# buttomnutstoast/Multigrid-Neural-Architectures

Hardware: NVIDIA B200
Metric: R-MG-34 train images/sec (higher is better)
Workload: dtype bf16

## Files before the change

include/mgconv.h:

```cpp
#ifndef MGCONV_H
#define MGCONV_H

#include <stdint.h>
#include <stddef.h>

#ifdef __cplusplus
extern "C" {
#endif

enum {
  MG_MAX_SEG = 6,
  MG_MAX_SRC = 8
};

typedef struct mg_ctx mg_ctx;

typedef enum {
  MG_OK = 0,
  MG_ERR_INVALID_ARG = 1,
  MG_ERR_SHAPE = 2,
  MG_ERR_CUDA = 3,
  MG_ERR_NCCL = 4,
  MG_ERR_UNSUPPORTED = 5
} mg_status;

typedef enum { MG_F32 = 0, MG_BF16 = 1 } mg_dtype;

typedef enum {
  MG_SEG_SAME = 0,
  MG_SEG_POOL = 1,
  MG_SEG_UP = 2
} mg_seg_mode;

typedef enum { MG_IMPL_AUTO = 0, MG_IMPL_SIMT = 1, MG_IMPL_TCGEN05 = 2 } mg_impl;

typedef struct { int64_t hi, lo; } mg_sum;

typedef struct {
  void* data;
  const float* scale;
  const float* shift;
  int32_t relu;
  int32_t N, H, W, C, Cp;
} mg_grid;

typedef struct {
  int32_t n_seg;
  mg_grid seg[MG_MAX_SEG];
  int32_t seg_mode[MG_MAX_SEG];
  int32_t ksize, stride, pad;
  int32_t Cout;
  int32_t H, W;
  int32_t algo_fwd, algo_bwd_data;
} mg_conv_desc;
enum { MG_ALGO_AUTO = 0, MG_ALGO_TILE128 = 1,
       MG_ALGO_TILE256 = 2,
       MG_ALGO_RESIDENT = 3,
       MG_ALGO_TILE128_DEEP = 4,
       MG_ALGO_TILE256_DEEP = 5,
       MG_ALGO_TILE128_MID = 6,
       MG_ALGO_PAIR128 = 7,
       MG_ALGO_PAIR256 = 8,
       MG_ALGO_RESIDENT_PAIR = 9 };

typedef struct {
  mg_grid g;
  int32_t c_offset;
  int32_t mode;
  const void* aux;
} mg_grad_src;

int mg_ctx_create(int device, void* cuda_stream, int dtype, mg_ctx** out);
int mg_ctx_destroy(mg_ctx* ctx);
int mg_ctx_set_stream(mg_ctx* ctx, void* cuda_stream);
int mg_ctx_set_impl(mg_ctx* ctx, int impl);
int mg_ctx_lane(mg_ctx* ctx, int lane);
int mg_ctx_event_record(mg_ctx* ctx, int ev);
int mg_ctx_event_wait(mg_ctx* ctx, int ev);
int mg_ctx_sync(mg_ctx* ctx);
enum { MG_TUNE_HALO_SUBTILES = 0,
       MG_TUNE_PERSISTENT = 1,
       MG_TUNE_STEM_FUSED_STATS = 2  };
int mg_ctx_set_tuning(mg_ctx* ctx, int knob, int value);
const char* mg_last_error(mg_ctx* ctx);
int mg_version(void);
int mg_ctx_launch_count(mg_ctx* ctx, int64_t* out);
int mg_ctx_tc_launch_count(mg_ctx* ctx, int64_t* out);
int mg_ctx_profile(mg_ctx* ctx, int on);
int mg_ctx_profile_read(mg_ctx* ctx, double* conv_ms, int64_t* conv_calls);

int mg_import_nchw(mg_ctx* ctx, const float* src, mg_grid* dst);
int mg_export_nchw(mg_ctx* ctx, const mg_grid* src, float* dst);

int mg_crop_flip_normalize(mg_ctx* ctx, const float* src, int32_t N, int32_t C, int32_t H, int32_t W, float* dst, int32_t oH, int32_t oW,
                           const int32_t* y0, const int32_t* x0, const int32_t* flip, const float* mean, const float* stdv);

size_t mg_conv_packed_bytes(const mg_conv_desc* d, int transposed);
int mg_conv_pack_weights(mg_ctx* ctx, const mg_conv_desc* d, const float* w, void* wpack, int transposed);
int mg_conv_pack_weights_batched(mg_ctx* ctx, int32_t n, const mg_conv_desc* const* descs, const float* const* w,
                                 void* const* wpack, const int32_t* transposed);

int mg_conv_forward(mg_ctx* ctx, const mg_conv_desc* d, const float* w, const void* wpack,
                    const float* bias, mg_grid* y, mg_sum* bn_sums);

int mg_bn_finalize(mg_ctx* ctx, const mg_sum* bn_sums, int64_t count, int32_t C, int32_t Cp,
                   const float* gamma, const float* beta, float* running_mean, float* running_var,
                   float eps, float momentum, int training,
                   float* scale, float* shift, float* save_mean, float* save_invstd);

int mg_residual_forward(mg_ctx* ctx, const mg_grid* z, const mg_grid* s, int relu, mg_grid* out, mg_grid* pooled);

typedef struct {
  const mg_sum* sums;
  int64_t count;
  const float* gamma;
  const float* beta;
// ... 89 lines not shown
```

multigrid-neural-architectures_b200/csrc/umma_conv.cu:

```cuda
#include "common.cuh"
#include "conv_view.cuh"
#include "umma_common.cuh"
#include "tma.cuh"
#include <algorithm>
#include <vector>

namespace {

constexpr int BM = 128;
constexpr int KV_PER_STAGE = 8;
constexpr int A_STAGE_BYTES = BM * 128;
constexpr int N_PRODUCERS = 128;
constexpr int MMA_WARP = 4, B_WARP = 5;
constexpr int N_THREADS = 192;
constexpr int MAX_STAGES = 8;

struct UParams {
  USeg seg[MG_MAX_SEG];
  int n_seg;
  int k, stride, pad;
  int H, W;
  int Ho, Wo;
  int64_t M;
  int Nimg;
// ... 266 lines not shown
      if (leader) tc_commit(&tmem_full_bar);
    }
  }
  __syncthreads();
  if (warp == MMA_WARP) {
    tc_fence_after();
    asm volatile("tcgen05.dealloc.cta_group::1.sync.aligned.b32 %0, %1;" ::"r"(tmem_base), "r"(p.tmem_cols) : "memory");
  }
}



__device__ __forceinline__ float warp_reduce_scatter16(float (&v)[16], int lane) {
#pragma unroll
  for (int o = 8; o >= 1; o >>= 1) {
    const bool hi = (lane & o) != 0;
#pragma unroll
    for (int i = 0; i < o; ++i) {
      const float send = hi ? v[i] : v[i + o];
      const float keep = hi ? v[i + o] : v[i];
      v[i] = keep + __shfl_xor_sync(0xffffffffu, send, o);
    }
  }
  return v[0] + __shfl_xor_sync(0xffffffffu, v[0], 16);
}

constexpr int MAX_CHUNKS = 32;
struct HChunk { int seg, c0, nch, tps, ksteps, stage0; };

struct HParams {
  CUtensorMap tmap[MG_MAX_SEG];
  int seg_up[MG_MAX_SEG];
  HChunk chunk[MAX_CHUNKS];
  int n_seg, n_chunks, n_stages, any_up;
  int img_box;
  int H, W, Wp, Hp, Nimg;
  int64_t T;
  int HL;
  int nr_max;
  int halo_bytes;
  int n_abuf;
  int n_tile;
  const uint8_t* wpack;
  const float* bias;
  int c_bias;
  __nv_bfloat16* y;
  int y_pitch, c_valid;
  int stages, tmem_cols;
  mg_sum* stats;
  int c_stats;
  int m_tiles;
  CUtensorMap tmap_w;
  int tile_rows;
  int epi_stage;
};

__device__ __forceinline__ void zero_pad_column(uint8_t* a_smem, int nbuf, int halo_bytes, int nr_max, int Wp, int tid, int nthreads, int org = 0) {
  for (int i = tid; i < nbuf * nr_max * 8; i += nthreads) {
    const int q = i & 7, row = (i >> 3) % nr_max, buf = (i >> 3) / nr_max;
    *reinterpret_cast<uint4*>(a_smem + (size_t)buf * halo_bytes + (size_t)(org + row * Wp + Wp - 1) * 128 + q * 16) = make_uint4(0, 0, 0, 0);
  }
  fence_proxy_async();
}

__device__ __forceinline__ void zero_halo_margins(uint8_t* a_smem, int nbuf, int halo_bytes, int HL, int Wp, int tid, int nthreads) {
  const int m = Wp + 1;
  for (int i = tid; i < nbuf * 2 * m * 8; i += nthreads) {
    const int q = i & 7, sl = (i >> 3) % (2 * m), buf = (i >> 3) / (2 * m);
    const int slot = sl < m ? sl : HL - 2 * m + sl;
    *reinterpret_cast<uint4*>(a_smem + (size_t)buf * halo_bytes + (size_t)slot * 128 + q * 16) = make_uint4(0, 0, 0, 0);
  }
  fence_proxy_async();
}

__device__ __forceinline__ bool slot_pixel(const HParams& p, int64_t t, uint32_t* pix) {
  if (t >= p.T) return false;
  const uint32_t tu = (uint32_t)t, spi = (uint32_t)(p.Hp * p.Wp);
  const uint32_t n = tu / spi, rem = tu - n * spi;
  const uint32_t yy = rem / (uint32_t)p.Wp, xs = rem - yy * (uint32_t)p.Wp;
  if ((int)yy >= p.H || (int)xs >= p.W) return false;
  *pix = (n * p.H + yy) * p.W + xs;
  return true;
}

template <int MT>
__global__ void __launch_bounds__(32 * (4 * MT + 3), MT == 1 ? 4 : 2) umma_conv_halo_kernel(const __grid_constant__ HParams p) {
  constexpr int EPI_WARPS = 4 * MT, A_WARP = EPI_WARPS, B_WARP = EPI_WARPS + 1, M_WARP = EPI_WARPS + 2, NT = 32 * (EPI_WARPS + 3);
  extern __shared__ __align__(1024) uint8_t smem_raw[];
  uint8_t* smem = (uint8_t*)(((uintptr_t)smem_raw + 1023) & ~(uintptr_t)1023);
  __shared__ uint64_t full_bar[MAX_STAGES], empty_bar[MAX_STAGES], a_full[2], a_empty[2], tmem_full_bar;
  __shared__ uint32_t tmem_base_s;
  __shared__ float s_bias[256];

  pdl_launch();
  const int tid = threadIdx.x, warp = tid >> 5, lane = tid & 31;
  const int S = p.stages;
  const int b_stage_bytes = p.n_tile * 128;
  uint8_t* a_smem = smem;
  uint8_t* b_smem = smem + (size_t)p.n_abuf * p.halo_bytes;
  const int t0 = (int)blockIdx.x * (BM * MT);
  const int ntile = blockIdx.y;
  const int hs = t0 - p.Wp - 1;
  const int r0 = floordiv(hs, p.Wp);
  const int nr = (hs + p.HL - 1) / p.Wp - r0 + 1;
  const int off = p.img_box ? 0 : hs - r0 * p.Wp;

// ... 319 lines not shown
      }
    }
  } else if (rank == 0) {
    const bool leader = elect_one();
    const uint32_t idesc = (1u << 4) | (1u << 7) | (1u << 10) | ((uint32_t)(p.n_tile >> 3) << 17) | ((uint32_t)(256 >> 4) << 24);
    Ring ra(p.n_abuf), rb(S);
    for (int c = 0; c < p.n_chunks; ++c, ra.next()) {
      const int buf = ra.idx;
      const HChunk ch = p.chunk[c];
      mbar_wait_cluster(&a_full[buf], ra.phase);
      tc_fence_after();
      const uint32_t a_base = smem_u32(a_smem + (size_t)buf * p.halo_bytes) + (uint32_t)a_first * 128u;
      const int tps = ch.tps, ksteps = ch.ksteps;
      const uint32_t sub_lo = 8u / (uint32_t)tps;
      int sub = 0;
      uint32_t b_lo = 0;
      for (int tap = 0; tap < 9; ++tap) {
        if (sub == 0) {
          mbar_wait_cluster(&full_bar[rb.idx], rb.phase);
          tc_fence_after();
          b_lo = desc_lo_k_sw128(smem_u32(b_smem + (size_t)rb.idx * b_half_bytes));
        }
        const uint32_t a_lo = desc_lo_k_sw128(a_base + (uint32_t)((tap / 3) * p.Wp + (tap % 3)) * 128u);
        const bool last_of_stage = (sub == tps - 1) || tap == 8;
        if (leader) {
#pragma unroll
          for (int mt = 0; mt < MT; ++mt)
#pragma unroll
            for (int q = 0; q < 4; ++q)
              if (q < ksteps) {
                tc_mma_bf16_lohi_pair(tmem_base + (uint32_t)(mt * p.n_tile), a_lo + (uint32_t)(mt * BM * 8 + q * 2), b_lo + (uint32_t)sub * sub_lo + (uint32_t)(q * 2),
                                      DESC_HI_SW128, idesc, (uint32_t)((c | tap | q) != 0));
              }
          if (last_of_stage) tc_commit_pair(&empty_bar[rb.idx]);
        }
        if (last_of_stage) { sub = 0; rb.next(); } else ++sub;
      }
      if (leader) tc_commit_pair(&a_empty[buf]);
    }
    if (leader) tc_commit_pair(&tmem_full_bar);
  }
  __syncthreads();
  cluster_sync_all();
  if (warp == M_WARP) {
    tc_fence_after();
    asm volatile("tcgen05.dealloc.cta_group::2.sync.aligned.b32 %0, %1;" ::"r"(tmem_base), "r"(p.tmem_cols) : "memory");
  }
}


constexpr int P_A_WARP = 8, P_B_WARP = 9, P_MMA_WARP = 10, P_THREADS = 352;
constexpr int P_MAX_ABUF = 6;

__global__ void __launch_bounds__(P_THREADS, 1) umma_conv_halo_persistent_kernel(const __grid_constant__ HParams p) {
  pdl_launch();
  extern __shared__ __align__(1024) uint8_t smem_raw[];
  uint8_t* smem = (uint8_t*)(((uintptr_t)smem_raw + 1023) & ~(uintptr_t)1023);
  __shared__ uint64_t b_full, a_full[P_MAX_ABUF], a_empty[P_MAX_ABUF], tmem_full[2], tmem_empty[2];
  __shared__ uint32_t tmem_base_s;

  const int tid = threadIdx.x, warp = tid >> 5, lane = tid & 31;
  const int NA = p.n_abuf;
  const int b_stage_bytes = p.n_tile * 128;
  uint8_t* a_smem = smem;
  uint8_t* b_smem = smem + (size_t)NA * p.halo_bytes;
  long long* s_part = reinterpret_cast<long long*>(b_smem + (size_t)p.n_stages * b_stage_bytes);
  float* s_bias = reinterpret_cast<float*>(s_part + 32 * p.n_tile);
  const int n_my = (p.m_tiles - (int)blockIdx.x + (int)gridDim.x - 1) / (int)gridDim.x;
  const int R = p.tile_rows;
  const int tile_slots = R ? R * p.Wp : BM;

  for (int c = tid; c < 32 * p.n_tile; c += P_THREADS) s_part[c] = 0;
  if (tid == 0) {
    mbar_init(&b_full, 1);
    for (int s = 0; s < NA; ++s) { mbar_init(&a_full[s], 1); mbar_init(&a_empty[s], 1); }
    for (int s = 0; s < 2; ++s) { mbar_init(&tmem_full[s], 1); mbar_init(&tmem_empty[s], 128); }
    asm volatile("fence.mbarrier_init.release.cluster;" ::: "memory");
  }
  if (warp == P_MMA_WARP) {
    asm volatile("tcgen05.alloc.cta_group::1.sync.aligned.shared::cta.b32 [%0], %1;" ::"r"(smem_u32(&tmem_base_s)), "r"(p.tmem_cols)
                 : "memory");
    asm volatile("tcgen05.relinquish_alloc_permit.cta_group::1.sync.aligned;" ::: "memory");
  }
  if (warp == P_A_WARP && lane < p.n_seg) tma_prefetch_desc(&p.tmap[lane]);
  if (p.img_box) zero_halo_margins(a_smem, NA, p.halo_bytes, p.HL, p.Wp, tid, P_THREADS);
  else if (p.any_up) zero_pad_column(a_smem, NA, p.halo_bytes, p.nr_max, p.Wp, tid, P_THREADS, R ? 1 : 0);
  if (R) {
    for (int i = tid; i < NA * 2 * 8; i += P_THREADS) {
      const int q = i & 7, which = (i >> 3) & 1, buf = i >> 4;
      const int slot = which ? 1 + (R + 2) * p.Wp : 0;
      *reinterpret_cast<uint4*>(a_smem + (size_t)buf * p.halo_bytes + (size_t)slot * 128 + q * 16) = make_uint4(0, 0, 0, 0);
    }
    fence_proxy_async();
  }
  pdl_wait();
  for (int c = tid; c < p.n_tile; c += P_THREADS) s_bias[c] = (p.bias && c < p.c_bias) ? p.bias[c] : 0.f;
  tc_fence_before();
  __syncthreads();
  tc_fence_after();
  const uint32_t tmem_base = tmem_base_s;

  if (warp < 8) {
    const int grp = warp >> 2, qw = warp & 3;
    const bool want_stats = p.stats != nullptr;
#ifdef MG_PHASE_PROF
    long long e_wait = 0, e_work = 0;
#endif
    for (int it = grp; it < n_my; it += 2) {
      const int mt = blockIdx.x + it * gridDim.x;
      const int acc = it & 1;
      const int row = qw * 32 + lane;
      uint32_t pix = 0;
      const bool row_ok = row < tile_slots && slot_pixel(p, (int64_t)mt * tile_slots + row, &pix);
#ifdef MG_PHASE_PROF
      const long long e0 = clock64();
#endif
      mbar_wait(&tmem_full[acc], (it >> 1) & 1);
      tc_fence_after();
#ifdef MG_PHASE_PROF
      const long long e1 = clock64();
#endif
      __nv_bfloat16* yrow = p.y + (size_t)pix * p.y_pitch;
      const uint32_t tcol = tmem_base + ((uint32_t)(qw * 32) << 16) + (uint32_t)(acc * p.n_tile);
      for (int c0 = 0; c0 < p.n_tile; c0 += 16) {
        uint32_t a16[16];
        tc_ld16(tcol + (uint32_t)c0, a16);
        tc_wait_ld();
        uint32_t pk[2][4];
#pragma unroll
        for (int h = 0; h < 2; ++h) {
          const int n0 = c0 + h * 8;
#pragma unroll
          for (int e = 0; e < 4; ++e) {
            const float a = __uint_as_float(a16[h * 8 + 2 * e]) + s_bias[c0 + h * 8 + 2 * e];
            const float b = __uint_as_float(a16[h * 8 + 2 * e + 1]) + s_bias[c0 + h * 8 + 2 * e + 1];
            __nv_bfloat162 t2 = __floats2bfloat162_rn(a, b);
            pk[h][e] = *reinterpret_cast<uint32_t*>(&t2);
          }
          if (row_ok && n0 + 8 <= p.c_valid) *reinterpret_cast<uint4*>(yrow + n0) = make_uint4(pk[h][0], pk[h][1], pk[h][2], pk[h][3]);
        }
        if (want_stats) {
#pragma unroll
          for (int h = 0; h < 2; ++h) {
            const bool use = row_ok && c0 + h * 8 + 8 <= p.c_valid;
            float sv[16];
#pragma unroll
            for (int e = 0; e < 4; ++e) {
              const float ra = use ? __uint_as_float(pk[h][e] << 16) : 0.f, rb = use ? __uint_as_float(pk[h][e] & 0xFFFF0000u) : 0.f;
              sv[2 * e] = ra; sv[2 * e + 1] = rb;
              sv[8 + 2 * e] = ra * ra; sv[8 + 2 * e + 1] = rb * rb;
            }
            const float tot = warp_reduce_scatter16(sv, lane);
            if (lane < 16) {
              long long fh, fl;
              mg_to_fix_f32(tot, fh, fl);
              long long* sp = s_part + (size_t)((warp * 2 + (lane >> 3)) * p.n_tile + c0 + h * 8 + (lane & 7)) * 2;
              sp[0] += fh; sp[1] += fl;
            }
          }
        }
      }
      tc_fence_before();
      mbar_arrive(&tmem_empty[acc]);
#ifdef MG_PHASE_PROF
      e_wait += e1 - e0; e_work += clock64() - e1;
#endif
    }
#ifdef MG_PHASE_PROF
    if (blockIdx.x == 3 && tid == 0) printf("epilogue warp0: tiles %d wait_tmem_full %lld work %lld cycles/tile\n", n_my, e_wait / n_my, e_work / n_my);
#endif
    if (want_stats) {
      asm volatile("bar.sync 3, 256;" ::: "memory");
      for (int c = tid; c < p.n_tile; c += 256)
        if (c < p.c_stats) {
          long long ah = 0, al = 0, bh = 0, bl = 0;
#pragma unroll
          for (int w = 0; w < 8; ++w) {
            const long long* sa = s_part + (size_t)((w * 2) * p.n_tile + c) * 2;
            const long long* sb = s_part + (size_t)((w * 2 + 1) * p.n_tile + c) * 2;
            ah += sa[0]; al += sa[1]; bh += sb[0]; bl += sb[1];
          }
          mg_sum_add_fix(p.stats + c, ah, al);
          mg_sum_add_fix(p.stats + p.c_stats + c, bh, bl);
        }
    }
  } else if (warp == P_A_WARP) {
    Ring ra(NA);
    int ac = 0;
    for (int it = 0; it < n_my; ++it) {
      const int t0 = (int)(blockIdx.x + it * gridDim.x) * tile_slots;
      const int hs = t0 - p.Wp - 1;
      const int r0 = R ? t0 / p.Wp - 1 : floordiv(hs, p.Wp);
      const int nr = R ? R + 2 : (hs + p.HL - 1) / p.Wp - r0 + 1;
      for (int c = 0; c < p.n_chunks; ++c, ++ac, ra.next()) {
        const int buf = ra.idx;
        if (ac >= NA) mbar_wait(&a_empty[buf], ra.phase ^ 1u);
        const HChunk ch = p.chunk[c];
        const uint32_t dst = smem_u32(a_smem + (size_t)buf * p.halo_bytes) + (R ? 128u : 0u);
        if (p.img_box) tma_load_images(&p.tmap[ch.seg], dst + (uint32_t)(p.Wp + 1) * 128u, &a_full[buf], ch.c0, t0 / (p.Hp * p.Wp), (uint32_t)BM * 128u, lane);
        else tma_load_rows(&p.tmap[ch.seg], p.seg_up[ch.seg], dst, &a_full[buf], ch.c0, r0, nr, p.W, p.Hp, lane);
      }
    }
  } else if (warp == P_B_WARP) {
    if (lane == 0) {
      mbar_arrive_expect_tx(&b_full, (uint32_t)(p.n_stages * b_stage_bytes));
      for (int q = 0; q < p.n_stages; ++q)
        bulk_g2s(smem_u32(b_smem + (size_t)q * b_stage_bytes), p.wpack + (size_t)q * b_stage_bytes, (uint32_t)b_stage_bytes, &b_full);
    }
  } else {
    const bool leader = elect_one();
    const uint32_t idesc = idesc_bf16_m128(p.n_tile);
    const uint32_t b_base = smem_u32(b_smem);
    Ring ra(NA);
    mbar_wait(&b_full, 0);
#ifdef MG_PHASE_PROF
    long long m_wait_e = 0, m_wait_a = 0, m_issue = 0, m_t0 = clock64();
#endif
    for (int it = 0; it < n_my; ++it) {
      const int acc = it & 1;
#ifdef MG_PHASE_PROF
      const long long q0 = clock64();
#endif
      if (it >= 2) { mbar_wait(&tmem_empty[acc], ((it >> 1) - 1) & 1); tc_fence_after(); }
#ifdef MG_PHASE_PROF
      m_wait_e += clock64() - q0;
#endif
      const uint32_t d_tmem = tmem_base + (uint32_t)(acc * p.n_tile);
      const int t0 = (int)(blockIdx.x + it * gridDim.x) * tile_slots;
      const int hs = t0 - p.Wp - 1;
      const int off = (p.img_box || R) ? 0 : hs - floordiv(hs, p.Wp) * p.Wp;
      for (int c = 0; c < p.n_chunks; ++c, ra.next()) {
        const int buf = ra.idx;
        const HChunk ch = p.chunk[c];
#ifdef MG_PHASE_PROF
        const long long q1 = clock64();
#endif
        mbar_wait(&a_full[buf], ra.phase);
        tc_fence_after();
#ifdef MG_PHASE_PROF
        const long long q2 = clock64();
        m_wait_a += q2 - q1;
#endif
        const uint32_t a_base = smem_u32(a_smem + (size_t)buf * p.halo_bytes) + (uint32_t)off * 128u;
        const int tps = ch.tps, ksteps = ch.ksteps;
        const uint32_t sub_lo = 8u / (uint32_t)tps;
        if (leader) {
          int sub = 0, st = ch.stage0;
          for (int tap = 0; tap < 9; ++tap) {
            const uint32_t a_lo = desc_lo_k_sw128(a_base + (uint32_t)((tap / 3) * p.Wp + (tap % 3)) * 128u);
            const uint32_t b_lo = desc_lo_k_sw128(b_base + (uint32_t)(st * b_stage_bytes)) + (uint32_t)sub * sub_lo;
#pragma unroll
            for (int q = 0; q < 4; ++q)
              if (q < ksteps) tc_mma_bf16_lohi(d_tmem, a_lo + (uint32_t)(q * 2), b_lo + (uint32_t)(q * 2), DESC_HI_SW128, idesc, (uint32_t)((c | tap | q) != 0));
            if (++sub == tps) { sub = 0; ++st; }
          }
          tc_commit(&a_empty[buf]);
        }
#ifdef MG_PHASE_PROF
        m_issue += clock64() - q2;
#endif
      }
      if (leader) tc_commit(&tmem_full[acc]);
    }
#ifdef MG_PHASE_PROF
    if (blockIdx.x == 3 && lane == 0) printf("MMA warp: tiles %d total %lld wait_tmem_empty %lld wait_a_full %lld issue %lld cycles/tile\n", n_my, (clock64() - m_t0) / n_my, m_wait_e / n_my, m_wait_a / n_my, m_issue / n_my);
#endif
  }
  __syncthreads();
  if (warp == P_MMA_WARP) {
    tc_fence_after();
    asm volatile("tcgen05.dealloc.cta_group::1.sync.aligned.b32 %0, %1;" ::"r"(tmem_base), "r"(p.tmem_cols) : "memory");
  }
}


__global__ void __cluster_dims__(2, 1, 1) __launch_bounds__(P_THREADS, 1) umma_conv_halo_persistent_pair_kernel(const __grid_constant__ HParams p) {
  pdl_launch();
  extern __shared__ __align__(1024) uint8_t smem_raw[];
  uint8_t* smem = (uint8_t*)(((uintptr_t)smem_raw + 1023) & ~(uintptr_t)1023);
  __shared__ uint64_t b_full, a_full[P_MAX_ABUF], a_empty[P_MAX_ABUF], tmem_full[2], tmem_empty[2];
  __shared__ uint32_t tmem_base_s;
// ... 696 lines not shown
    p.stages = S;
    const int smem = p.n_abuf * p.halo_bytes + S * half + 1024;
    MG_REQUIRE(ctx, smem <= SMEM_MAX, MG_ERR_UNSUPPORTED, "pair halo conv: %d bytes of shared memory", smem);
    p.epi_stage = epilogue_staging(p, MT, smem - 1024);
    int rc = mg_tensor_map(ctx, p.wpack, g.n_tiles * p.n_stages * p.n_tile, 0, 0, 0, 5, p.n_tile / 2, &p.tmap_w);
    if (rc) return rc;
    static bool pair_attr_set = false;
    if (!pair_attr_set) {
      MG_CUDA(ctx, cudaFuncSetAttribute(umma_conv_halo_pair_kernel<1>, cudaFuncAttributeMaxDynamicSharedMemorySize, SMEM_MAX));
      MG_CUDA(ctx, cudaFuncSetAttribute(umma_conv_halo_pair_kernel<2>, cudaFuncAttributeMaxDynamicSharedMemorySize, SMEM_MAX));
      pair_attr_set = true;
    }
    dim3 grid((unsigned)mg_round_up((int)mg_cdiv(p.T, BM * MT), 2), (unsigned)g.n_tiles);
    if (MT == 2) MG_CUDA(ctx, mg_launch_pdl(umma_conv_halo_pair_kernel<2>, grid, dim3(32 * 11), (size_t)smem, ctx->stream, p));
    else MG_CUDA(ctx, mg_launch_pdl(umma_conv_halo_pair_kernel<1>, grid, dim3(32 * 7), (size_t)smem, ctx->stream, p));
    MG_CHECK_LAUNCH(ctx);
    ctx->tc_launches++;
    return MG_OK;
  }
  int budget_kb;
  if (MT == 1) {
    budget_kb = p.n_tile >= 192 ? 108 : 56;
  } else {
    const int ctas = std::max(1, std::min(512 / cols, 2));
    budget_kb = ctas == 1 ? 200 : 108;
  }
  if (algo == MG_ALGO_TILE128_MID) budget_kb = 72;
  if ((algo == MG_ALGO_AUTO || algo == MG_ALGO_RESIDENT) && mg_cdiv(p.T, BM * MT) * g.n_tiles <= ctx->num_sms) budget_kb = 200;
  if (algo == MG_ALGO_TILE128_DEEP) budget_kb = 108;
  if (algo == MG_ALGO_TILE256_DEEP) budget_kb = 200;
  if (budget_env > 0) budget_kb = budget_env;
  const int min_ring = 2;
  p.n_abuf = (g.n_chunks > 1 && 2 * p.halo_bytes + min_ring * b_stage <= budget_kb * 1024) ? 2 : 1;
  int S = (budget_kb * 1024 - p.n_abuf * p.halo_bytes) / b_stage;
  S = std::max(2, std::min(S, std::min(MAX_STAGES, p.n_stages)));
  p.stages = S;
  static bool attr_set = false;
  if (!attr_set) {
    MG_CUDA(ctx, cudaFuncSetAttribute(umma_conv_halo_kernel<1>, cudaFuncAttributeMaxDynamicSharedMemorySize, SMEM_MAX));
    MG_CUDA(ctx, cudaFuncSetAttribute(umma_conv_halo_kernel<2>, cudaFuncAttributeMaxDynamicSharedMemorySize, SMEM_MAX));
    attr_set = true;
  }
  const int smem = p.n_abuf * p.halo_bytes + S * b_stage + 1024;
  MG_REQUIRE(ctx, smem <= SMEM_MAX, MG_ERR_UNSUPPORTED, "halo conv: %d bytes of shared memory", smem);
  p.epi_stage = epilogue_staging(p, MT, smem - 1024);
  dim3 grid((unsigned)mg_cdiv(p.T, BM * MT), (unsigned)g.n_tiles);
  if (MT == 2) MG_CUDA(ctx, mg_launch_pdl(umma_conv_halo_kernel<2>, grid, dim3(32 * 11), (size_t)smem, ctx->stream, p));
  else MG_CUDA(ctx, mg_launch_pdl(umma_conv_halo_kernel<1>, grid, dim3(32 * 7), (size_t)smem, ctx->stream, p));
  MG_CHECK_LAUNCH(ctx);
  ctx->tc_launches++;
  return MG_OK;
}

struct PersistPlan { int n_abuf, smem, tmem_cols, grid, tile_rows, halo_bytes, pair; };
static int persist_tile_rows(const mg_conv_desc* d, int Nimg, bool any_up) {
  const int Wp = d->W + 1, Hp = d->H + 1;
  if (Wp > BM) return 0;
  if (!any_up && BM % (Hp * Wp) == 0) return 0;
  const int R = BM / Wp;
  if (R < 1 || R * Wp * 100 < BM * 85) return 0;
  (void)Nimg;
  return R;
}
static bool persist_plan(const mg_ctx* ctx, const mg_conv_desc* d, const Geometry& g, int Nimg, int algo, bool stats, PersistPlan* pl) {
  static int on = -1, min_tiles_per_sm = -1;
  if (on < 0) { const char* e = getenv("MGCONV_PERSIST"); on = e ? atoi(e) : 1; }
  if (min_tiles_per_sm < 0) { const char* e = getenv("MGCONV_PERSIST_MIN_TILES"); min_tiles_per_sm = e ? atoi(e) : 4; }
  if (algo == MG_ALGO_TILE128 || algo == MG_ALGO_TILE256 || algo == MG_ALGO_TILE128_DEEP || algo == MG_ALGO_TILE256_DEEP ||
      algo == MG_ALGO_TILE128_MID || algo == MG_ALGO_PAIR128 || algo == MG_ALGO_PAIR256) return false;
  const bool pair = algo == MG_ALGO_RESIDENT_PAIR;
  const bool forced = algo == MG_ALGO_RESIDENT || pair || ctx->tune_persist == 1;
  if (!forced && (ctx->tune_persist == 2 || !on)) return false;
  if (!g.halo || g.n_tiles != 1) return false;
  HParams hp;
  hp.Wp = d->W + 1; hp.img_box = 0;
  halo_geometry(hp, BM);
  bool any_up = false;
  for (int s = 0; s < d->n_seg; ++s) any_up = any_up || d->seg_mode[s] == MG_SEG_UP;
  static int aligned_single = -1;
  if (aligned_single < 0) { const char* e = getenv("MGCONV_PERSIST_ALIGNED"); aligned_single = e ? atoi(e) : 0; }
  const int R = ((pair || aligned_single) && !stats) ? persist_tile_rows(d, Nimg, any_up && g.n_chunks > 0) : 0;
  if (R) hp.halo_bytes = mg_round_up(((R + 2) * hp.Wp + 2) * 128, 1024);
  const int64_t m_tiles = R ? mg_cdiv((int64_t)Nimg * (d->H + 1), R) : mg_cdiv((int64_t)Nimg * (d->H + 1) * hp.Wp, BM);
  if (!forced && m_tiles < (int64_t)min_tiles_per_sm * ctx->num_sms) return false;
  if (pair && !R && !(!any_up && BM % ((d->H + 1) * hp.Wp) == 0)) return false;
  const int b_bytes = g.n_stages * g.n_tile * (pair ? 64 : 128);
  const int tail = g.n_tile * (4 + 256);
  const int room = SMEM_MAX - 1024 - b_bytes - tail;
  int n_abuf = room / hp.halo_bytes;
  if (n_abuf < 2) return false;
  n_abuf = std::min(n_abuf, std::min(P_MAX_ABUF, 2 * g.n_chunks + 1));
  int cols = 32;
  while (cols < 2 * g.n_tile) cols <<= 1;
  if (cols > 512) return false;
  pl->n_abuf = n_abuf; pl->smem = n_abuf * hp.halo_bytes + b_bytes + tail + 1024; pl->tmem_cols = cols;
  pl->grid = (int)std::min<int64_t>(m_tiles, ctx->num_sms);
  if (pair) pl->grid = 2 * (int)std::min<int64_t>((m_tiles + 1) / 2, ctx->num_sms / 2);
  pl->tile_rows = R; pl->halo_bytes = hp.halo_bytes; pl->pair = pair ? 1 : 0;
  return true;
}

static int launch_halo_persistent(mg_ctx* ctx, HParams& p, const PersistPlan& pl, const mg_grid* segs) {
  { int rc = halo_tensor_maps(ctx, p, segs, BM); if (rc) return rc; }
  halo_geometry(p, BM);
  p.m_tiles = (int)mg_cdiv(p.T, BM);
  p.tile_rows = p.img_box ? 0 : pl.tile_rows;
  if (p.tile_rows) {
    p.halo_bytes = pl.halo_bytes;
    p.nr_max = p.tile_rows + 2;
    p.m_tiles = (int)mg_cdiv((int64_t)p.Nimg * p.Hp, p.tile_rows);
  }
  p.tmem_cols = pl.tmem_cols;
  p.n_abuf = pl.n_abuf;
  p.stages = 0;
  static bool attr_set = false;
  if (!attr_set) {
    MG_CUDA(ctx, cudaFuncSetAttribute(umma_conv_halo_persistent_kernel, cudaFuncAttributeMaxDynamicSharedMemorySize, SMEM_MAX));
    attr_set = true;
  }
  if (pl.pair) {
    int rc = mg_tensor_map(ctx, p.wpack, p.n_stages * p.n_tile, 0, 0, 0, 5, p.n_tile / 2, &p.tmap_w);
    if (rc) return rc;
    static bool pair_attr = false;
    if (!pair_attr) {
      MG_CUDA(ctx, cudaFuncSetAttribute(umma_conv_halo_persistent_pair_kernel, cudaFuncAttributeMaxDynamicSharedMemorySize, SMEM_MAX));
      pair_attr = true;
    }
    MG_CUDA(ctx, mg_launch_pdl(umma_conv_halo_persistent_pair_kernel, dim3(pl.grid), dim3(P_THREADS), (size_t)pl.smem, ctx->stream, p));
    MG_CHECK_LAUNCH(ctx);
    ctx->tc_launches++;
    return MG_OK;
  }
  MG_CUDA(ctx, mg_launch_pdl(umma_conv_halo_persistent_kernel, dim3(pl.grid), dim3(P_THREADS), (size_t)pl.smem, ctx->stream, p));
  MG_CHECK_LAUNCH(ctx);
  ctx->tc_launches++;
  return MG_OK;
}

static bool fused_stats_on() {
  static int on = -1;
  if (on < 0) { const char* e = getenv("MGCONV_FUSED_STATS"); on = e ? atoi(e) : 1; }
  return on != 0;
}

static int fill_halo_params(mg_ctx* ctx, HParams& p, const Geometry& g, int n_seg, const mg_grid* segs, const int* up, int N, int H, int W) {
  memset(&p, 0, sizeof(p));
  p.n_seg = n_seg; p.n_chunks = g.n_chunks; p.n_stages = g.n_stages;
  for (int c = 0; c < g.n_chunks; ++c) p.chunk[c] = g.chunk[c];
  p.H = H; p.W = W; p.Wp = W + 1; p.Hp = H + 1; p.Nimg = N;
  p.T = (int64_t)N * p.Hp * p.Wp;
  p.n_tile = g.n_tile;
  for (int s = 0; s < n_seg; ++s) {
    p.seg_up[s] = up[s];
    if (up[s]) p.any_up = 1;
  }
  return MG_OK;
}

}

bool umma_wgrad_supported(const mg_ctx* ctx, const mg_conv_desc* d);

bool umma_conv_supported(const mg_ctx* ctx, const mg_conv_desc* d, int kind) {
  if (ctx->dtype != MG_BF16) return false;
  if (kind == 2) return umma_wgrad_supported(ctx, d);
  if (kind == 1 && d->stride != 1) return false;
// ... 195 lines not shown
```

multigrid-neural-architectures_b200/mgconv/ffi.py:

```python
import ctypes as C
import os

MG_MAX_SEG = 6
MG_MAX_SRC = 8
MG_F32, MG_BF16 = 0, 1
MG_SEG_SAME, MG_SEG_POOL, MG_SEG_UP, MG_SRC_POOL3 = 0, 1, 2, 3
MG_IMPL_AUTO, MG_IMPL_SIMT, MG_IMPL_TCGEN05 = 0, 1, 2
MG_TUNE_HALO_SUBTILES, MG_TUNE_PERSISTENT, MG_TUNE_STEM_FUSED_STATS = 0, 1, 2
MG_ALGO_AUTO, MG_ALGO_TILE128, MG_ALGO_TILE256, MG_ALGO_RESIDENT, MG_ALGO_TILE128_DEEP, MG_ALGO_TILE256_DEEP, MG_ALGO_TILE128_MID = 0, 1, 2, 3, 4, 5, 6
MG_ALGO_PAIR128, MG_ALGO_PAIR256, MG_ALGO_RESIDENT_PAIR = 7, 8, 9

_HERE = os.path.dirname(os.path.abspath(__file__))
LIB_PATH = os.environ.get("MGCONV_LIB", os.path.join(_HERE, "libmgconv.so"))


class MGError(RuntimeError):
    pass


class mg_grid(C.Structure):
    _fields_ = [("data", C.c_void_p), ("scale", C.c_void_p), ("shift", C.c_void_p), ("relu", C.c_int32),
                ("N", C.c_int32), ("H", C.c_int32), ("W", C.c_int32), ("C", C.c_int32), ("Cp", C.c_int32)]


class mg_conv_desc(C.Structure):
    _fields_ = [("n_seg", C.c_int32), ("seg", mg_grid * MG_MAX_SEG), ("seg_mode", C.c_int32 * MG_MAX_SEG),
                ("ksize", C.c_int32), ("stride", C.c_int32), ("pad", C.c_int32), ("Cout", C.c_int32),
                ("H", C.c_int32), ("W", C.c_int32), ("algo_fwd", C.c_int32), ("algo_bwd_data", C.c_int32)]


class mg_grad_src(C.Structure):
    _fields_ = [("g", mg_grid), ("c_offset", C.c_int32), ("mode", C.c_int32), ("aux", C.c_void_p)]


MG_STAGE_MAX_GRIDS = 4


class mg_stage_desc(C.Structure):
    _fields_ = [("n_scales", C.c_int32), ("C_in", C.c_int32 * MG_STAGE_MAX_GRIDS), ("C_out", C.c_int32 * MG_STAGE_MAX_GRIDS),
                ("H", C.c_int32 * MG_STAGE_MAX_GRIDS), ("W", C.c_int32 * MG_STAGE_MAX_GRIDS), ("ksize", C.c_int32 * MG_STAGE_MAX_GRIDS),
                ("residual", C.c_int32), ("no_final_relu", C.c_int32), ("eps", C.c_float), ("momentum", C.c_float)]


class mg_stage_params(C.Structure):
    _fields_ = [(name, C.c_void_p * (2 * MG_STAGE_MAX_GRIDS)) for name in
                ("conv_w", "conv_b", "bn_g", "bn_b", "bn_rm", "bn_rv", "conv_gw", "conv_gb", "bn_gg", "bn_gb")]


class mg_bn_fused(C.Structure):
    _fields_ = [("sums", C.c_void_p), ("count", C.c_int64), ("gamma", C.c_void_p), ("beta", C.c_void_p),
                ("running_mean", C.c_void_p), ("running_var", C.c_void_p), ("eps", C.c_float), ("momentum", C.c_float),
                ("training", C.c_int32), ("save_mean", C.c_void_p), ("save_invstd", C.c_void_p)]


def _load():
    if not os.path.exists(LIB_PATH):
        raise MGError(
            f"{LIB_PATH} not found: build it with `make -C multigrid-neural-architectures_b200/csrc` "
            "(or __graft_entry__.build()); there is no CPU / PyTorch fallback for the multigrid hot path")
    return C.CDLL(LIB_PATH, mode=C.RTLD_GLOBAL)


lib = _load()
# ... 135 lines not shown
```

multigrid-neural-architectures_b200/mgconv/ops.py:

```python
import ctypes as C
import os
import torch

from . import ffi
from .ffi import mg_grid, mg_conv_desc, mg_grad_src, mg_bn_fused, ptr, MG_SEG_SAME, MG_SEG_POOL, MG_SEG_UP, MG_SRC_POOL3, MG_MAX_SRC


def cpad(c):
    return (c + 7) // 8 * 8


def _k(x):
    if x is None:
        return None
    if isinstance(x, torch.Tensor):
        return x.data_ptr()
    if isinstance(x, mg_grid):
        return x.data
    return int(x)


def _keys(*xs):
    return [k for k in (_k(x) for x in xs) if k]

# ... 176 lines not shown
        d = mg_conv_desc()
        d.n_seg = len(self.segs)
        for i, (t, m) in enumerate(self.segs):
            d.seg[i] = t.grid()
            d.seg_mode[i] = m
        d.ksize, d.stride, d.pad, d.Cout, d.H, d.W = self.k, self.stride, self.pad, self.Cout, self.H, self.W
        self.desc = d
        self.y.buf = E.alloc(self.y.shape())
        self.yg = self.y.grid()
        if self.want_stats:
            self.sums = E.alloc_sums(2 * self.Cout, "fwd")
        t0 = self.segs[0][0]
        self.col = None
        if (E.use_packed and len(self.segs) == 1 and self.segs[0][1] == MG_SEG_SAME and self.stride > 1 and self.k > 1
                and t0.C * self.k * self.k <= 512 and not t0.needs_grad and os.environ.get("MGCONV_STEM_IM2COL", "0") == "1"):
            K = t0.C * self.k * self.k
            Kp = cpad(K)
            self.col = E.alloc((self.y.N, self.Ho, self.Wo, Kp))
            self.col_g = mg_grid(self.col.data_ptr(), None, None, 0, self.y.N, self.Ho, self.Wo, K, Kp)
            self.in_g = t0.grid()
            d1 = mg_conv_desc()
            d1.n_seg = 1
            d1.seg[0] = self.col_g
            d1.seg_mode[0] = MG_SEG_SAME
            d1.ksize, d1.stride, d1.pad, d1.Cout, d1.H, d1.W = 1, 1, 0, self.Cout, self.Ho, self.Wo
            self.desc_direct, self.desc = d, d1
        self.wpack = self.wpack_t = None
        nb = ffi.lib.mg_conv_packed_bytes(C.byref(self.desc), 0) if E.use_packed else 0
        if nb:
            self.wpack = E.alloc((nb,), torch.uint8)
        self.Ccat = sum(t.C for t, _ in self.segs)
        self.CcatP = sum(t.Cp for t, _ in self.segs)

    def pack(self, E):
        if self.wpack is not None:
            E.ctx.call("mg_conv_pack_weights", C.byref(self.desc), ptr(self.mod.weight), ptr(self.wpack), 0)
        if self.wpack_t is not None:
            E.ctx.call("mg_conv_pack_weights", C.byref(self.desc), ptr(self.mod.weight), ptr(self.wpack_t), 1)

    def pack_jobs(self):
        jobs = []
        if self.wpack is not None:
            jobs.append((self.desc, self.mod.weight, self.wpack, 0))
        if self.wpack_t is not None:
            jobs.append((self.desc, self.mod.weight, self.wpack_t, 1))
        return jobs

    def _tunable(self):
        return self.wpack is not None and self.k == 3 and self.stride == 1 and self.pad == 1 and 7 <= self.W <= 63

    def _pick(self, E, field, run):
        best, best_t = 0, None
        for algo in (ffi.MG_ALGO_TILE128, ffi.MG_ALGO_TILE256, ffi.MG_ALGO_RESIDENT, ffi.MG_ALGO_TILE128_DEEP, ffi.MG_ALGO_TILE256_DEEP,
                     ffi.MG_ALGO_TILE128_MID, ffi.MG_ALGO_PAIR128, ffi.MG_ALGO_PAIR256, ffi.MG_ALGO_RESIDENT_PAIR):
            setattr(self.desc, field, algo)
            run()
            e0, e1 = torch.cuda.Event(enable_timing=True), torch.cuda.Event(enable_timing=True)
            e0.record()
            for _ in range(3):
                run()
            e1.record()
            e1.synchronize()
            t = e0.elapsed_time(e1)
            if best_t is None or t < best_t * 0.97:
                best, best_t = algo, t
        setattr(self.desc, field, best)
        return best

    def tune_fwd(self, E):
        if self._tunable():
            self._pick(E, "algo_fwd", lambda: self.fwd(E))

    def tune_bwd(self, E):
        if self._tunable() and self.needs_dgrad and self.wpack_t is not None:
            g = self.y.G
            self._pick(E, "algo_bwd_data", lambda: E.ctx.call("mg_conv_backward_data", C.byref(self.desc), ptr(self.mod.weight),
                                                              ptr(self.wpack_t), C.byref(g), C.byref(self.dcat_g)))

    def size(self):
        return self.H

    def io_fwd(self):
        return _keys(*[t.buf for t, _ in self.segs]), _keys(self.y.buf, self.sums, self.col)

    def io_bwd(self):
        io = self.ycomb.io() if self.ycomb is not None else None
        r = _keys(self.y.G, self.col, *[t.buf for t, _ in self.segs])
        w = _keys(self.mod.gradWeight, self.mod.gradBias, self.dcat)
        return _merge(io, (r, w))

    def fwd(self, E):
        if self.col is not None:
            E.ctx.call("mg_im2col", C.byref(self.in_g), self.k, self.stride, self.pad, C.byref(self.col_g))
        E.ctx.call("mg_conv_forward", C.byref(self.desc), ptr(self.mod.weight), ptr(self.wpack), ptr(self.mod.bias),
                   C.byref(self.yg), ptr(self.sums))

    def setup_bwd(self, E):
        if self.apply is None:
            self.ycomb = Combine(E, self.y)
            self.y.G = self.ycomb.grid()
        self.needs_dgrad = any(t.needs_grad for t, _ in self.segs)
        self.dcat = None
        if self.needs_dgrad:
            self.dcat = E.alloc((self.y.N, self.H, self.W, self.CcatP))
            self.dcat_g = mg_grid(self.dcat.data_ptr(), None, None, 0, self.y.N, self.H, self.W, self.CcatP, self.CcatP)
            off = 0
            for t, m in self.segs:
# ... 460 lines not shown
```

Baseline: 15420.

## Add narrow resident conv algo with two CTAs per SM and contiguous tiles

Adds a new MG_ALGO_RESIDENT_NARROW persistent halo conv variant for layers with small packed weights. It sizes shared memory so two CTAs can co-reside per SM (launch bounds raised to 2), skips the stats scratch when stats are off, and assigns each CTA a contiguous range of M tiles instead of a strided one. The autotuner picks it per layer only when it measures faster, so other layers are unaffected. Raising the launch bound to 2 also applies to the existing persistent path and may constrain registers there.

```diff
diff --git a/include/mgconv.h b/include/mgconv.h
--- a/include/mgconv.h
+++ b/include/mgconv.h
@@ -61,7 +61,8 @@
        MG_ALGO_TILE128_MID = 6,
        MG_ALGO_PAIR128 = 7,
        MG_ALGO_PAIR256 = 8,
-       MG_ALGO_RESIDENT_PAIR = 9 };
+       MG_ALGO_RESIDENT_PAIR = 9,
+       MG_ALGO_RESIDENT_NARROW = 10 };
 
 typedef struct {
   mg_grid g;
diff --git a/multigrid-neural-architectures_b200/csrc/umma_conv.cu b/multigrid-neural-architectures_b200/csrc/umma_conv.cu
--- a/multigrid-neural-architectures_b200/csrc/umma_conv.cu
+++ b/multigrid-neural-architectures_b200/csrc/umma_conv.cu
@@ -342,6 +342,7 @@
   int m_tiles;
   CUtensorMap tmap_w;
   int tile_rows;
+  int tile_contig;
   int epi_stage;
 };
 
@@ -767,7 +768,7 @@
 constexpr int P_A_WARP = 8, P_B_WARP = 9, P_MMA_WARP = 10, P_THREADS = 352;
 constexpr int P_MAX_ABUF = 6;
 
-__global__ void __launch_bounds__(P_THREADS, 1) umma_conv_halo_persistent_kernel(const __grid_constant__ HParams p) {
+__global__ void __launch_bounds__(P_THREADS, 2) umma_conv_halo_persistent_kernel(const __grid_constant__ HParams p) {
   pdl_launch();
   extern __shared__ __align__(1024) uint8_t smem_raw[];
   uint8_t* smem = (uint8_t*)(((uintptr_t)smem_raw + 1023) & ~(uintptr_t)1023);
@@ -780,12 +781,17 @@
   uint8_t* a_smem = smem;
   uint8_t* b_smem = smem + (size_t)NA * p.halo_bytes;
   long long* s_part = reinterpret_cast<long long*>(b_smem + (size_t)p.n_stages * b_stage_bytes);
-  float* s_bias = reinterpret_cast<float*>(s_part + 32 * p.n_tile);
-  const int n_my = (p.m_tiles - (int)blockIdx.x + (int)gridDim.x - 1) / (int)gridDim.x;
+  float* s_bias = reinterpret_cast<float*>(s_part + (p.stats ? 32 * p.n_tile : 0));
+  const int G = (int)gridDim.x, bx = (int)blockIdx.x;
+  const int per = p.m_tiles / G, extra = p.m_tiles % G;
+  const int first = p.tile_contig ? bx * per + min(bx, extra) : bx;
+  const int step = p.tile_contig ? 1 : G;
+  const int n_my = p.tile_contig ? per + (bx < extra ? 1 : 0) : (p.m_tiles - bx + G - 1) / G;
   const int R = p.tile_rows;
   const int tile_slots = R ? R * p.Wp : BM;
 
-  for (int c = tid; c < 32 * p.n_tile; c += P_THREADS) s_part[c] = 0;
+  if (p.stats)
+    for (int c = tid; c < 32 * p.n_tile; c += P_THREADS) s_part[c] = 0;
   if (tid == 0) {
     mbar_init(&b_full, 1);
     for (int s = 0; s < NA; ++s) { mbar_init(&a_full[s], 1); mbar_init(&a_empty[s], 1); }
@@ -822,7 +828,7 @@
     long long e_wait = 0, e_work = 0;
 #endif
     for (int it = grp; it < n_my; it += 2) {
-      const int mt = blockIdx.x + it * gridDim.x;
+      const int mt = first + it * step;
       const int acc = it & 1;
       const int row = qw * 32 + lane;
       uint32_t pix = 0;
@@ -903,7 +909,7 @@
     Ring ra(NA);
     int ac = 0;
     for (int it = 0; it < n_my; ++it) {
-      const int t0 = (int)(blockIdx.x + it * gridDim.x) * tile_slots;
+      const int t0 = (first + it * step) * tile_slots;
       const int hs = t0 - p.Wp - 1;
       const int r0 = R ? t0 / p.Wp - 1 : floordiv(hs, p.Wp);
       const int nr = R ? R + 2 : (hs + p.HL - 1) / p.Wp - r0 + 1;
@@ -941,7 +947,7 @@
       m_wait_e += clock64() - q0;
 #endif
       const uint32_t d_tmem = tmem_base + (uint32_t)(acc * p.n_tile);
-      const int t0 = (int)(blockIdx.x + it * gridDim.x) * tile_slots;
+      const int t0 = (first + it * step) * tile_slots;
       const int hs = t0 - p.Wp - 1;
       const int off = (p.img_box || R) ? 0 : hs - floordiv(hs, p.Wp) * p.Wp;
       for (int c = 0; c < p.n_chunks; ++c, ra.next()) {
@@ -1744,7 +1750,7 @@
   return MG_OK;
 }
 
-struct PersistPlan { int n_abuf, smem, tmem_cols, grid, tile_rows, halo_bytes, pair; };
+struct PersistPlan { int n_abuf, smem, tmem_cols, grid, tile_rows, halo_bytes, pair, contig; };
 static int persist_tile_rows(const mg_conv_desc* d, int Nimg, bool any_up) {
   const int Wp = d->W + 1, Hp = d->H + 1;
   if (Wp > BM) return 0;
@@ -1754,6 +1760,27 @@
   (void)Nimg;
   return R;
 }
+constexpr int NARROW_MAX_WEIGHTS = 72 * 1024;
+constexpr int NARROW_CTA_SMEM = 233472 / 2 - 1024 - 2048;
+static bool narrow_plan(const mg_ctx* ctx, const mg_conv_desc* d, const Geometry& g, int Nimg, bool stats, int halo_bytes, PersistPlan* pl) {
+  const int b_bytes = g.n_stages * g.n_tile * 128;
+  if (b_bytes > NARROW_MAX_WEIGHTS) return false;
+  const int tail = g.n_tile * (4 + (stats ? 256 : 0));
+  const int fixed = b_bytes + tail + 1024;
+  int ctas = 2, n_abuf = (NARROW_CTA_SMEM - fixed) / halo_bytes;
+  if (n_abuf < 2) { ctas = 1; n_abuf = 2; }
+  if (n_abuf * halo_bytes + fixed > SMEM_MAX) return false;
+  n_abuf = std::min(n_abuf, std::min(P_MAX_ABUF, 2 * g.n_chunks + 1));
+  int cols = 32;
+  while (cols < 2 * g.n_tile) cols <<= 1;
+  if (cols > 256) return false;
+  const int64_t m_tiles = mg_cdiv((int64_t)Nimg * (d->H + 1) * (d->W + 1), BM);
+  pl->n_abuf = n_abuf; pl->smem = n_abuf * halo_bytes + fixed; pl->tmem_cols = cols;
+  pl->grid = (int)std::min<int64_t>(m_tiles, ctas * ctx->num_sms);
+  pl->tile_rows = 0; pl->halo_bytes = halo_bytes; pl->pair = 0; pl->contig = 1;
+  return true;
+}
+
 static bool persist_plan(const mg_ctx* ctx, const mg_conv_desc* d, const Geometry& g, int Nimg, int algo, bool stats, PersistPlan* pl) {
   static int on = -1, min_tiles_per_sm = -1;
   if (on < 0) { const char* e = getenv("MGCONV_PERSIST"); on = e ? atoi(e) : 1; }
@@ -1762,11 +1789,12 @@
       algo == MG_ALGO_TILE128_MID || algo == MG_ALGO_PAIR128 || algo == MG_ALGO_PAIR256) return false;
   const bool pair = algo == MG_ALGO_RESIDENT_PAIR;
   const bool forced = algo == MG_ALGO_RESIDENT || pair || ctx->tune_persist == 1;
-  if (!forced && (ctx->tune_persist == 2 || !on)) return false;
+  if (algo != MG_ALGO_RESIDENT_NARROW && !forced && (ctx->tune_persist == 2 || !on)) return false;
   if (!g.halo || g.n_tiles != 1) return false;
   HParams hp;
   hp.Wp = d->W + 1; hp.img_box = 0;
   halo_geometry(hp, BM);
+  if (algo == MG_ALGO_RESIDENT_NARROW) return narrow_plan(ctx, d, g, Nimg, stats, hp.halo_bytes, pl);
   bool any_up = false;
   for (int s = 0; s < d->n_seg; ++s) any_up = any_up || d->seg_mode[s] == MG_SEG_UP;
   static int aligned_single = -1;
@@ -1788,7 +1816,7 @@
   pl->n_abuf = n_abuf; pl->smem = n_abuf * hp.halo_bytes + b_bytes + tail + 1024; pl->tmem_cols = cols;
   pl->grid = (int)std::min<int64_t>(m_tiles, ctx->num_sms);
   if (pair) pl->grid = 2 * (int)std::min<int64_t>((m_tiles + 1) / 2, ctx->num_sms / 2);
-  pl->tile_rows = R; pl->halo_bytes = hp.halo_bytes; pl->pair = pair ? 1 : 0;
+  pl->tile_rows = R; pl->halo_bytes = hp.halo_bytes; pl->pair = pair ? 1 : 0; pl->contig = 0;
   return true;
 }
 
@@ -1804,6 +1832,7 @@
   }
   p.tmem_cols = pl.tmem_cols;
   p.n_abuf = pl.n_abuf;
+  p.tile_contig = pl.contig;
   p.stages = 0;
   static bool attr_set = false;
   if (!attr_set) {
diff --git a/multigrid-neural-architectures_b200/mgconv/ffi.py b/multigrid-neural-architectures_b200/mgconv/ffi.py
--- a/multigrid-neural-architectures_b200/mgconv/ffi.py
+++ b/multigrid-neural-architectures_b200/mgconv/ffi.py
@@ -8,7 +8,7 @@
 MG_IMPL_AUTO, MG_IMPL_SIMT, MG_IMPL_TCGEN05 = 0, 1, 2
 MG_TUNE_HALO_SUBTILES, MG_TUNE_PERSISTENT, MG_TUNE_STEM_FUSED_STATS = 0, 1, 2
 MG_ALGO_AUTO, MG_ALGO_TILE128, MG_ALGO_TILE256, MG_ALGO_RESIDENT, MG_ALGO_TILE128_DEEP, MG_ALGO_TILE256_DEEP, MG_ALGO_TILE128_MID = 0, 1, 2, 3, 4, 5, 6
-MG_ALGO_PAIR128, MG_ALGO_PAIR256, MG_ALGO_RESIDENT_PAIR = 7, 8, 9
+MG_ALGO_PAIR128, MG_ALGO_PAIR256, MG_ALGO_RESIDENT_PAIR, MG_ALGO_RESIDENT_NARROW = 7, 8, 9, 10
 
 _HERE = os.path.dirname(os.path.abspath(__file__))
 LIB_PATH = os.environ.get("MGCONV_LIB", os.path.join(_HERE, "libmgconv.so"))
diff --git a/multigrid-neural-architectures_b200/mgconv/ops.py b/multigrid-neural-architectures_b200/mgconv/ops.py
--- a/multigrid-neural-architectures_b200/mgconv/ops.py
+++ b/multigrid-neural-architectures_b200/mgconv/ops.py
@@ -252,7 +252,8 @@
     def _pick(self, E, field, run):
         best, best_t = 0, None
         for algo in (ffi.MG_ALGO_TILE128, ffi.MG_ALGO_TILE256, ffi.MG_ALGO_RESIDENT, ffi.MG_ALGO_TILE128_DEEP, ffi.MG_ALGO_TILE256_DEEP,
-                     ffi.MG_ALGO_TILE128_MID, ffi.MG_ALGO_PAIR128, ffi.MG_ALGO_PAIR256, ffi.MG_ALGO_RESIDENT_PAIR):
+                     ffi.MG_ALGO_TILE128_MID, ffi.MG_ALGO_PAIR128, ffi.MG_ALGO_PAIR256, ffi.MG_ALGO_RESIDENT_PAIR,
+                     ffi.MG_ALGO_RESIDENT_NARROW):
             setattr(self.desc, field, algo)
             run()
             e0, e1 = torch.cuda.Event(enable_timing=True), torch.cuda.Event(enable_timing=True)
diff --git a/scratch/narrow_layers.py b/scratch/narrow_layers.py
--- /dev/null
+++ b/scratch/narrow_layers.py
@@ -0,0 +1,130 @@
+import ctypes as C
+import collections
+import json
+import os
+import sys
+
+ROOT = os.path.dirname(os.path.dirname(os.path.abspath(__file__)))
+sys.path.insert(0, ROOT); sys.path.insert(0, os.path.join(ROOT, "multigrid-neural-architectures_b200")); sys.path.insert(0, os.path.join(ROOT, "tests"))
+import torch
+from mgconv import ffi
+from mgconv.ffi import ptr, MG_SEG_SAME, MG_SEG_UP
+from util import Grid, conv_desc
+
+N = 256
+SHAPES = {
+    "b1 28x28 112->32": (28, [(64, "s"), (32, "s"), (16, "u")], 32),
+    "b1 14x14 48->16": (14, [(32, "s"), (16, "s")], 16),
+    "b2 7x7 96->32": (7, [(64, "s"), (32, "s")], 32),
+}
+
+
+def cp8(c):
+    return (c + 7) // 8 * 8
+
+
+def work(H, segs, Cout):
+    cin = sum(c for c, _ in segs)
+    flops = 2.0 * N * H * H * Cout * cin * 9
+    x_bytes = sum(N * (H // 2 if m == "u" else H) ** 2 * cp8(c) * 2 for c, m in segs)
+    y_bytes = N * H * H * cp8(Cout) * 2
+    dcat_bytes = N * H * H * sum(cp8(c) for c, _ in segs) * 2
+    return flops, {"fwd": x_bytes + y_bytes, "dgrad": y_bytes + dcat_bytes}
+
+
+def micro(algos):
+    ctx = ffi.Context(0, torch.cuda.current_stream().cuda_stream, ffi.MG_BF16)
+    flush = torch.empty(256 << 20, dtype=torch.uint8, device="cuda")
+    for name, (H, segs, Cout) in SHAPES.items():
+        gs, modes = [], []
+        for c, m in segs:
+            g = Grid(ffi.MG_BF16, N, c, H // 2 if m == "u" else H, H // 2 if m == "u" else H)
+            g.t.normal_()
+            gs.append(g); modes.append(MG_SEG_UP if m == "u" else MG_SEG_SAME)
+        d = conv_desc(gs, modes, 3, 1, 1, Cout, H, H)
+        w = torch.randn(Cout, sum(c for c, _ in segs), 3, 3, device="cuda") * 0.05
+        b = torch.zeros(Cout, device="cuda")
+        wp = torch.zeros(ffi.lib.mg_conv_packed_bytes(C.byref(d), 0), dtype=torch.uint8, device="cuda")
+        wpt = torch.zeros(ffi.lib.mg_conv_packed_bytes(C.byref(d), 1), dtype=torch.uint8, device="cuda")
+        ctx.call("mg_conv_pack_weights", C.byref(d), ptr(w), ptr(wp), 0)
+        ctx.call("mg_conv_pack_weights", C.byref(d), ptr(w), ptr(wpt), 1)
+        y = Grid(ffi.MG_BF16, N, Cout, H, H)
+        g = Grid(ffi.MG_BF16, N, Cout, H, H); g.t.normal_()
+        cp = sum(x.Cp for x in gs)
+        dcat = Grid(ffi.MG_BF16, N, cp, H, H, Cp=cp)
+        sums = torch.zeros(4 * Cout, dtype=torch.int64, device="cuda")
+        flops, nbytes = work(H, segs, Cout)
+        calls = {
+            "fwd": lambda: ctx.call("mg_conv_forward", C.byref(d), ptr(w), ptr(wp), ptr(b), C.byref(y.g()), ptr(sums)),
+            "dgrad": lambda: ctx.call("mg_conv_backward_data", C.byref(d), ptr(w), ptr(wpt), C.byref(g.g()), C.byref(dcat.g())),
+        }
+        print(f"{name}: packed weights fwd {wp.numel() / 1024:.1f} KB, dgrad {wpt.numel() / 1024:.1f} KB; "
+              f"{flops / 1e9:.2f} GFLOP; HBM fwd {nbytes['fwd'] / 1e6:.1f} MB, dgrad {nbytes['dgrad'] / 1e6:.1f} MB", flush=True)
+        for kind, f in calls.items():
+            row = []
+            for algo in algos:
+                d.algo_fwd = d.algo_bwd_data = algo
+                for _ in range(3):
+                    f()
+                torch.cuda.synchronize()
+                ts = []
+                for _ in range(30):
+                    flush.zero_()
+                    e0, e1 = torch.cuda.Event(enable_timing=True), torch.cuda.Event(enable_timing=True)
+                    e0.record(); f(); e1.record()
+                    torch.cuda.synchronize()
+                    ts.append(e0.elapsed_time(e1))
+                ts.sort()
+                us = ts[len(ts) // 2] * 1e3
+                row.append(f"algo {algo}: {us:6.1f} us {flops / us / 1e6:6.0f} TFLOP/s {nbytes[kind] / us / 1e6:5.2f} TB/s")
+            print(f"  {kind:5s}  " + "\n         ".join(row), flush=True)
+    ctx.close()
+
+
+def trace(out):
+    from torch.profiler import profile, ProfilerActivity
+    from mgconv import builders as B
+    net = B.load_net("ilsvrc/rnmg")
+    torch.manual_seed(2)
+    model = net.createModel(B.Opt(nGPU=1, depth=34)); model.precision = "bf16"; model.cuda()
+    crit = net.createCriterion()
+    params, grads = model.getParameters()
+    st = dict(learningRate=0.1, momentum=0.9, weightDecay=1e-4, dampening=0.0)
+    x = torch.randn(N, 3, 224, 224, device="cuda"); t = torch.randint(1, 1001, (N,), device="cuda")
+
+    def step():
+        model.zeroGradParameters()
+        net.btrain(params, lambda _p: (net.ftrain(x, t, model, crit)[1], grads), st)
+    for _ in range(4):
+        step()
+    torch.cuda.synchronize()
+    with profile(activities=[ProfilerActivity.CUDA]) as prof:
+        for _ in range(2):
+            step()
+        torch.cuda.synchronize()
+    tr = out + ".pt.trace.json"
+    prof.export_chrome_trace(tr)
+    ev = [e for e in json.load(open(tr))["traceEvents"] if e.get("cat") == "kernel"]
+    os.remove(tr)
+    groups = collections.defaultdict(list)
+    for e in ev:
+        nm = e["name"]
+        if "halo" not in nm or "wgrad" in nm:
+            continue
+        a = e.get("args", {})
+        key = (nm.replace("(anonymous namespace)::", "").split("(")[0], "x".join(map(str, a.get("grid", []))),
+               "x".join(map(str, a.get("block", []))), a.get("shared memory", 0))
+        groups[key].append(e["dur"])
+    with open(out, "w") as fo:
+        fo.write(f"{torch.cuda.get_device_name()}; halo fwd/dgrad launches of 2 laned R-MG-34 steps (B = {N}), torch.profiler CUDA activities\n")
+        fo.write(f"{'kernel':48s} {'grid':>8s} {'block':>6s} {'smem':>7s} {'n':>4s} {'avg us':>8s} {'total us':>9s}\n")
+        for k, v in sorted(groups.items(), key=lambda kv: -sum(kv[1])):
+            fo.write(f"{k[0]:48s} {k[1]:>8s} {k[2]:>6s} {k[3]:>7d} {len(v):4d} {sum(v) / len(v):8.1f} {sum(v):9.1f}\n")
+    print(open(out).read())
+
+
+if __name__ == "__main__":
+    if sys.argv[1] == "micro":
+        micro([int(a) for a in (sys.argv[2] if len(sys.argv) > 2 else "1,2,3,4,5,6,7,8,9").split(",")])
+    else:
+        trace(sys.argv[2])
```

New measurement: 15420 (median of 6 runs). About the same (+0.0%).
